# JuliaPhysics/BeamletOptics.jl

Hardware: AMD Instinct MI355X
Metric: ray-surface intersections/s (higher is better)
Workload: dtype f64

## Files before the change

### beamletoptics.jl_amd/csrc/bmo_lane.hpp

```cpp
#pragma once
#include <math.h>
#include <stdint.h>

#include "../../include/bmo.h"
#include "bmo_jlmath.hpp"

#if defined(__HIPCC__)
#define BMO_HD __host__ __device__ __forceinline__
#define BMO_NOUNROLL _Pragma("unroll 1")
#else
#define BMO_HD inline __attribute__((always_inline))
#define BMO_NOUNROLL
#endif

#if !defined(BMO_DUAL_PASSES)
#define BMO_DUAL_PASSES 1
#endif

namespace bmo {

#if defined(BMO_EMU_STATS)
inline long g_emu_sdf_any = 0, g_emu_sdf_leaf = 0, g_emu_normal = 0, g_emu_normal_fd = 0;
#endif

#if defined(__HIP_DEVICE_COMPILE__)
#define BMO_UNIFORM(i) __builtin_amdgcn_readfirstlane(i)
#define BMO_KONST __attribute__((address_space(4)))
__device__ __forceinline__ bool bmo_same_id(int32_t u, int32_t id) {
    asm volatile("" : "+s"(u));
    return u == id;
}
#else
#define BMO_UNIFORM(i) (i)
#define BMO_KONST
inline bool bmo_same_id(int32_t u, int32_t id) { return u == id; }
#endif
#if defined(__HIP_DEVICE_COMPILE__)
#define BMO_WAVE_ALL(p) (__all(p) != 0)
#define BMO_WAVE_ANY(p) (__any(p) != 0)
#else
#define BMO_WAVE_ALL(p) (p)
#define BMO_WAVE_ANY(p) (p)
#endif
typedef const BMO_KONST bmo_shape CShape;
typedef const BMO_KONST bmo_object CObject;
typedef const BMO_KONST double CDouble;
typedef const BMO_KONST int32_t CInt;


struct SceneView {
    CObject* objects;
    CShape* shapes;
    CInt* children;
    CDouble* tris;
    CDouble* n_table;
    CDouble* coefs;
    const BMO_KONST struct Cand* cands;
    int32_t n_objects, n_lambda, n_cands;
    double eps_srf, eps_ray, eps_ins, mt_keps, mt_leps, grad_h;
    int32_t march_iters;
    const BMO_KONST struct BvhNode* bvh_nodes = nullptr;
    CInt* bvh_faces = nullptr;
};

struct d3 {
    double x, y, z;
};
struct Hit {
    double t;
    d3 n;
    int32_t obj, shape;
};

BMO_HD double kinf() { return __builtin_huge_val(); }
BMO_HD bool sgn(double x) { return __builtin_signbit(x); }
BMO_HD bool isnan_(double x) { return x != x; }
BMO_HD Hit no_hit() {
    Hit h;
    h.t = kinf();
    h.n = {0, 0, 0};
    h.obj = -1;
    h.shape = -1;
    return h;
}

BMO_HD double jmax_rule(double x, double y) {
    if (isnan_(x) || isnan_(y)) return x + y;
    return ((y > x) || (sgn(y) < sgn(x))) ? y : x;
}
BMO_HD double jmin_rule(double x, double y) {
    if (isnan_(x) || isnan_(y)) return x + y;
    return ((y < x) || (sgn(y) > sgn(x))) ? y : x;
}
#if defined(__HIP_DEVICE_COMPILE__) && !defined(BMO_RULE_MINMAX)
BMO_HD double jmax(double x, double y) {
    double m;
    asm("v_max_f64 %0, %1, %2" : "=v"(m) : "v"(x), "v"(y));
    return __builtin_isunordered(x, y) ? x + y : m;
}
BMO_HD double jmin(double x, double y) {
    double m;
    asm("v_min_f64 %0, %1, %2" : "=v"(m) : "v"(x), "v"(y));
    return __builtin_isunordered(x, y) ? x + y : m;
}
#else
BMO_HD double jmax(double x, double y) { return jmax_rule(x, y); }
BMO_HD double jmin(double x, double y) { return jmin_rule(x, y); }
#endif
BMO_HD double jabs(double x) { return fabs(x); }
BMO_HD double jsqrt(double x) { return sqrt(x); }
BMO_HD double val(double x) { return x; }

template <int N>
struct DualN {
    double v;
    double p[N];
};
using Dual = DualN<3>;
#define BMO_DN template <int N> BMO_HD
BMO_DN double val(const DualN<N>& x) { return x.v; }
BMO_DN DualN<N> operator+(const DualN<N>& x, const DualN<N>& y) {
    DualN<N> r;
    r.v = x.v + y.v;
    for (int q = 0; q < N; ++q) r.p[q] = x.p[q] + y.p[q];
    return r;
}
BMO_DN DualN<N> operator-(const DualN<N>& x, const DualN<N>& y) {
    DualN<N> r;
    r.v = x.v - y.v;
    for (int q = 0; q < N; ++q) r.p[q] = x.p[q] - y.p[q];
    return r;
}
BMO_DN DualN<N> operator+(const DualN<N>& x, double c) {
    DualN<N> r = x;
    r.v = x.v + c;
    return r;
}
BMO_DN DualN<N> operator+(double c, const DualN<N>& x) {
    DualN<N> r = x;
    r.v = c + x.v;
    return r;
}
BMO_DN DualN<N> operator-(const DualN<N>& x, double c) {
    DualN<N> r = x;
    r.v = x.v - c;
    return r;
}
BMO_DN DualN<N> operator-(double c, const DualN<N>& x) {
    DualN<N> r;
    r.v = c - x.v;
    for (int q = 0; q < N; ++q) r.p[q] = -x.p[q];
    return r;
}
BMO_DN DualN<N> operator-(const DualN<N>& x) {
    DualN<N> r;
    r.v = -x.v;
    for (int q = 0; q < N; ++q) r.p[q] = -x.p[q];
    return r;
}
BMO_DN DualN<N> operator*(const DualN<N>& x, const DualN<N>& y) {
    DualN<N> r;
    r.v = x.v * y.v;
    for (int q = 0; q < N; ++q) r.p[q] = (x.p[q] * y.v) + (y.p[q] * x.v);
    return r;
}
BMO_DN DualN<N> operator*(const DualN<N>& x, double c) {
    DualN<N> r;
    r.v = x.v * c;
    for (int q = 0; q < N; ++q) r.p[q] = x.p[q] * c;
    return r;
}
BMO_DN DualN<N> operator*(double c, const DualN<N>& x) {
    DualN<N> r;
    r.v = c * x.v;
    for (int q = 0; q < N; ++q) r.p[q] = x.p[q] * c;
    return r;
}
BMO_DN DualN<N> operator/(const DualN<N>& x, double c) {
    DualN<N> r;
    r.v = x.v / c;
    for (int q = 0; q < N; ++q) r.p[q] = x.p[q] / c;
    return r;
}
BMO_DN DualN<N> jsqrt(const DualN<N>& x) {
    const double s = sqrt(x.v);
    const double d = 1.0 / (2.0 * s);
    DualN<N> r;
    r.v = s;
    for (int q = 0; q < N; ++q) r.p[q] = x.p[q] * d;
    return r;
}
BMO_DN DualN<N> jabs(const DualN<N>& x) {
    const bool neg = sgn(x.v);
    DualN<N> r;
    r.v = neg ? -x.v : x.v;
    for (int q = 0; q < N; ++q) r.p[q] = neg ? -x.p[q] : x.p[q];
    return r;
}
BMO_DN DualN<N> jmax(const DualN<N>& x, const DualN<N>& y) {
    const bool xw = x.v > y.v;
    DualN<N> r;
    r.v = xw ? x.v : y.v;
    for (int q = 0; q < N; ++q) r.p[q] = xw ? x.p[q] : y.p[q];
    return r;
}
BMO_DN DualN<N> jmin(const DualN<N>& x, const DualN<N>& y) {
    const bool xw = x.v < y.v;
    DualN<N> r;
    r.v = xw ? x.v : y.v;
    for (int q = 0; q < N; ++q) r.p[q] = xw ? x.p[q] : y.p[q];
    return r;
}
BMO_DN DualN<N> jmax(const DualN<N>& x, double y) {
    const bool xw = x.v > y;
    DualN<N> r;
    r.v = xw ? x.v : y;
    for (int q = 0; q < N; ++q) r.p[q] = xw ? x.p[q] : 0.0;
    return r;
}
BMO_DN DualN<N> jmin(const DualN<N>& x, double y) {
    const bool xw = x.v < y;
    DualN<N> r;
    r.v = xw ? x.v : y;
    for (int q = 0; q < N; ++q) r.p[q] = xw ? x.p[q] : 0.0;
    return r;
}

template <class T>
struct v3 {
    T x, y, z;
};

BMO_HD void pin(double& x) {
#if defined(__HIP_DEVICE_COMPILE__) && !defined(BMO_NO_PIN)
    asm volatile("" : "+v"(x));
#else
    (void)x;
#endif
}
template <int N>
BMO_HD void pin(DualN<N>& x) {
    pin(x.v);
}
template <class T>
BMO_HD void pin3(v3<T>& p) {
    pin(p.x);
    pin(p.y);
    pin(p.z);
}
BMO_HD double dot3(const d3& a, const d3& b) { return (a.x * b.x + a.y * b.y) + a.z * b.z; }
BMO_HD double norm3(const d3& a) { return sqrt(dot3(a, a)); }
BMO_HD d3 sub3(const d3& a, const d3& b) { return {a.x - b.x, a.y - b.y, a.z - b.z}; }
BMO_HD d3 neg3(const d3& a) { return {-a.x, -a.y, -a.z}; }
BMO_HD d3 cross3(const d3& a, const d3& b) { return {a.y * b.z - a.z * b.y, a.z * b.x - a.x * b.z, a.x * b.y - a.y * b.x}; }
BMO_HD d3 axpy3(const d3& p, double s, const d3& d) { return {p.x + s * d.x, p.y + s * d.y, p.z + s * d.z}; }
BMO_HD d3 normalize_div(const d3& a) {
    double n = norm3(a);
    return {a.x / n, a.y / n, a.z / n};
}
BMO_HD d3 normalize_inv(const d3& a) {
    double inv = 1.0 / norm3(a);
    return {a.x * inv, a.y * inv, a.z * inv};
}
template <class T>
BMO_HD T norm2(const T& x, const T& y) {
    return jsqrt(x * x + y * y);
}
template <class T>
BMO_HD T norm3t(const T& x, const T& y, const T& z) {
    return jsqrt((x * x + y * y) + z * z);
}

BMO_HD bool isapprox(double x, double y, double atol) {
    double rtol = atol > 0.0 ? 0.0 : 1.4901161193847656e-08;
    if (x == y) return true;
    if (isnan_(x) || isnan_(y) || fabs(x) == kinf() || fabs(y) == kinf()) return false;
    return fabs(x - y) <= fmax(atol, rtol * fmax(fabs(x), fabs(y)));
}

template <class T>
BMO_HD v3<T> to_local(CShape& s, const v3<T>& pt) {
    T dx = pt.x - s.pos[0], dy = pt.y - s.pos[1], dz = pt.z - s.pos[2];
    CDouble* m = s.tdir;
    return {(m[0] * dx + m[1] * dy) + m[2] * dz, (m[3] * dx + m[4] * dy) + m[5] * dz, (m[6] * dx + m[7] * dy) + m[8] * dz};
}

template <class T>
BMO_HD T slab2(const T& dx, const T& dy) {
    T mx = jmax(dx, dy);
    T ax = jmax(dx, 0.0), ay = jmax(dy, 0.0);
    return jmin(mx, 0.0) + norm2(ax, ay);
}


BMO_DN DualN<N> operator/(const DualN<N>& x, const DualN<N>& y) {
    const double ia = 1.0 / y.v, fb = -(x.v / (y.v * y.v));
    DualN<N> r;
    r.v = x.v / y.v;
    for (int q = 0; q < N; ++q) r.p[q] = (x.p[q] * ia) + (y.p[q] * fb);
    return r;
}
BMO_DN DualN<N> operator/(double x, const DualN<N>& y) {
    const double divv = x / y.v, f = -(divv / y.v);
    DualN<N> r;
    r.v = divv;
    for (int q = 0; q < N; ++q) r.p[q] = y.p[q] * f;
    return r;
}
BMO_HD bool lt(double a, double b) { return a < b; }
BMO_DN bool lt(const DualN<N>& a, double b) { return a.v < b; }
BMO_DN bool lt(double a, const DualN<N>& b) { return a < b.v; }
BMO_DN bool lt(const DualN<N>& a, const DualN<N>& b) { return a.v < b.v; }
BMO_HD double lit2(double x) { return x * x; }
BMO_HD double lit3(double x) { return x * x * x; }
BMO_DN DualN<N> lit2(const DualN<N>& x) {
    const double d = 2 * x.v;
    DualN<N> r;
    r.v = x.v * x.v;
    for (int q = 0; q < N; ++q) r.p[q] = x.p[q] * d;
    return r;
}
BMO_DN DualN<N> lit3(const DualN<N>& x) {
    const double d = 3 * (x.v * x.v);
    DualN<N> r;
    r.v = x.v * x.v * x.v;
    for (int q = 0; q < N; ++q) r.p[q] = x.p[q] * d;
    return r;
}
BMO_HD double ipow(double x, int n) {
    if (n == 0) return 1.0;
    if (n == 1) return x;
    if (n == 2) return x * x;
    if (n == 3) return x * x * x;
    double r = 1.0;
    while (n > 0) {
        if (n & 1) r *= x;
        x *= x;
        n >>= 1;
    }
    return r;
}
BMO_DN DualN<N> ipow(const DualN<N>& x, int n) {
    const double ev = ipow(x.v, n);
    const double f = n == 0 ? 0.0 : ipow(x.v, n - 1);
    DualN<N> r;
    r.v = ev;
    for (int q = 0; q < N; ++q) r.p[q] = (n == 0 || x.p[q] == 0) ? 0.0 : (x.p[q] * n) * f;
    return r;
}
BMO_HD double knan() { return kinf() - kinf(); }
BMO_HD double mknan(double) { return knan(); }
BMO_DN DualN<N> mknan(const DualN<N>&) {
    DualN<N> r;
    r.v = knan();
    for (int q = 0; q < N; ++q) r.p[q] = knan();
    return r;
}
BMO_HD double jsign(double x) { return x > 0 ? 1.0 : (x < 0 ? -1.0 : x); }
BMO_HD double clamp01(double x) { return x > 1.0 ? 1.0 : (x < 0.0 ? 0.0 : x); }
BMO_DN DualN<N> clamp01(const DualN<N>& x) {
    DualN<N> r = x;
    if (x.v > 1.0 || x.v < 0.0) {
        r.v = x.v > 1.0 ? 1.0 : 0.0;
        for (int q = 0; q < N; ++q) r.p[q] = 0.0;
    }
    return r;
}
template <class T>
BMO_HD void asph_eval(const T& r, double c, double k, CDouble* a, int na, T& z, T& g) {
    const T r2 = lit2(r);
    const T sa1 = 1 - (1 + k) * (c * c) * r2;
    const double Ri = 1 / c;
    const T sa2 = 1 - lit2(r) * (1 + k) / (Ri * Ri);
    T sum_a = r2 * 0.0, sum_r = r * 0.0;
    BMO_NOUNROLL
    for (int i = 1; i <= na; ++i) {
        const T ta = a[i - 1] * ipow(r2, i);
        const T tr = (2 * i * a[i - 1]) * ipow(r, 2 * (i - 1) + 1);
        sum_a = i == 1 ? ta : sum_a + ta;
        sum_r = i == 1 ? tr : sum_r + tr;
    }
    z = lt(sa1, 0.0) ? mknan(r) : c * r2 / (1 + jsqrt(sa1)) + sum_a;
    if (lt(sa2, 0.0)) {
        g = mknan(r);
    } else {
        const T sq = jsqrt(sa2);
        const T gr = 2 * r / (Ri * (sq + 1)) + lit3(r) * (1 + k) / ((Ri * Ri * Ri) * sq * lit2(sq + 1));
        g = -sum_r - gr;
    }
}
template <class T>
BMO_HD T norm_g(const T& g1) { return jsqrt(lit2(g1) + 1.0 * 1.0); }
template <class T>
BMO_HD T sd_line_segment(const T& px, const T& py, double ax, double ay, double bx, double by) {
    const T pax = px - ax, pay = py - ay;
    const double bax = bx - ax, bay = by - ay;
    const T h = clamp01((pax * bax + pay * bay) / (bax * bax + bay * bay));
    const T ex = pax - h * bax, ey = pay - h * bay;
    return jsqrt(ex * ex + ey * ey);
}
template <class T>
BMO_HD T asph_distance(bool convex, const T& r, const T& z, double c, double k, double d, CDouble* a, int na, double max_sag) {
    const T r2 = lit2(r);
    const double r2_bound = (d / 2) * (d / 2);
    T zv, g;
    double zb, gb;
    asph_eval<T>(r, c, k, a, na, zv, g);
    asph_eval<double>(d / 2, c, k, a, na, zb, gb);
    const T e = r - jsign(val(r)) * d / 2;
    const double ngb = norm_g<double>(gb);
    if (convex) {
        if (isnan_(val(zv)) || isnan_(val(g)) || lt(r2_bound, r2)) {
            T db;
            if (lt(z, zb)) db = jsqrt(lit2(e) + lit2(z - zb));
            else if (lt(zb, z) && lt(z, 0.0)) db = jsqrt(lit2(e));
            else if (lt(0.0, z) && (jsign(c) == 1 && zb < 0)) db = jsqrt(lit2(e) + lit2(z));
            else db = jsqrt(lit2(e) + lit2(z - zb));
            return db / ngb;
        }
        const T da = jabs(z - zv) / norm_g<T>(g);
        if (jsign(c) == 1 && zb < 0) {
            const T s1 = sd_line_segment<T>(r, z, d / 2, zb, d / 2, max_sag) / ngb;
            const T s2 = sd_line_segment<T>(r, z, d / 2, max_sag, -d / 2, max_sag) / ngb;
            const T s3 = sd_line_segment<T>(r, z, -d / 2, max_sag, -d / 2, zb) / ngb;
            const T m = jmin(jmin(jmin(da, s1), s2), s3);
            return (lt(zv, z) && lt(z, max_sag)) ? -m : m;
        }
        const T sdl = sd_line_segment<T>(r, z, d / 2, zb, -d / 2, zb) / ngb;
        if (lt(jsign(c) * zv, jsign(c) * z) && lt(jsign(c) * z, jsign(c) * zb)) return -jmin(sdl, da);
        return jmin(sdl, da);
    }
    if (isnan_(val(zv)) || isnan_(val(g))) {
        T db;
        if (lt(z, 0.0)) db = jsqrt(lit2(e) + lit2(z));
        else if (lt(0.0, z) && lt(z, zb)) db = jsqrt(lit2(e));
        else db = jsqrt(lit2(e) + lit2(z - zb));
        return db / ngb;
    }
    const T da = jabs(z - zv) / norm_g<T>(g);
    if (max_sag > 0 && zb < 0) {
        const T sdl = sd_line_segment<T>(r, z, d / 2, zb, -d / 2, zb) / ngb;
        if (lt(r2_bound, r2)) return sdl;
        if (lt(zb, z) && lt(z, zv)) return -jmin(da, sdl);
        if (zb > 0 && (lt(0.0, z) && lt(z, zv))) return -jmin(da, sdl);
        return jmin(da, sdl);
    }
    const T s1 = sd_line_segment<T>(r, z, d / 2, zb, d / 2, 0.0) / ngb;
    const T s2 = sd_line_segment<T>(r, z, d / 2, 0.0, -d / 2, 0.0) / ngb;
    const T s3 = sd_line_segment<T>(r, z, -d / 2, 0.0, -d / 2, zb) / ngb;
    if (lt(r2_bound, r2)) return jmin(jmin(s1, s2), s3);
    const T m = jmin(jmin(jmin(da, s1), s2), s3);
    if (zb < 0 && (lt(zv, z) && lt(z, 0.0))) return -m;
    if (zb > 0 && (lt(0.0, z) && lt(z, zv))) return -m;
    return m;
}
BMO_HD double asph_leaf(CShape& s, CDouble* coefs, double r, double y) {
    return asph_distance<double>(s.kind == BMO_SHAPE_ASPH_CONVEX, r, y, 1 / s.p[0], s.p[1], s.p[2], coefs + s.child_begin, s.child_count, s.p[3]);
}
BMO_DN DualN<N> asph_leaf(CShape&, CDouble*, const DualN<N>& r, const DualN<N>&) { return mknan(r); }

template <class T, int EXT>
BMO_HD T sdf_leaf(CShape& s, const int kind, const v3<T>& pt, CDouble* coefs) {
    const double P0 = s.p[0], P1 = s.p[1], P2 = s.p[2], P3 = s.p[3];
    v3<T> p = to_local(s, pt);
    const unsigned cls = (unsigned)((0x0005041214032150ull >> (4 * (kind & 15))) & 15ull) * (kind < 16 ? 1u : 0u);
    if (cls == 1) {
        pin3(p);
        double ra, ha, off, sub;
        if (kind == BMO_SHAPE_PLANO) {
            ra = P1 / 2;
            ha = P0 / 2;
            off = P0 / 2;
            sub = 0.0;
        } else if (kind == BMO_SHAPE_CYLINDER) {
            ra = P0;
            ha = P1;
            off = 0.0;
            sub = 0.0;
        } else {
            ra = P1;
            ha = P2;
            off = 0.0;
            sub = P0;
        }
        T r = norm2(p.x, p.z);
        if (kind == BMO_SHAPE_RING) r = r - sub;
        T h = kind == BMO_SHAPE_PLANO ? p.y - off : p.y;
        return slab2(jabs(r) - ra, jabs(h) - ha);
    }
    if (cls == 2) {
        pin3(p);
        double radius = P0, w, height;
        T q1 = norm2(p.x, p.z), q2;
        if (kind == BMO_SHAPE_CONVEX) {
            w = P1 / 2;
            height = P3;
            q2 = -p.y + radius;
        } else {
            height = P1;
            w = P2;
            q2 = p.y;
        }
        double a = val(q1), b = val(q2);
        double sv = jmax((height - radius) * (a * a) + (w * w) * (height + radius - 2 * b), height * a - w * b);
        if (sv < 0) return norm2(q1, q2) - radius;
        if (a < w) return height - q2;
        return norm2(q1 - w, q2 - height);
    }
    if (cls == 3) {
        pin3(p);
        double radius = P0, dia = P1, sag = P2;
        T x0 = p.x + 0.0, z0 = p.z + 0.0;
        T y1 = p.y + sag / 2;
        T r = norm2(x0, z0);
        T sdf1 = slab2(jabs(r) - dia / 2, jabs(y1) - sag / 2);
        T y2 = p.y + radius;
        T sdf2 = norm3t(x0, y2, z0) - radius;
        return jmax(sdf1, -sdf2);
    }
    if (cls == 4) {
        pin3(p);
        T qx = jabs(p.x) - P0, qy = jabs(p.y) - P1, qz = jabs(p.z) - P2;
        T box = norm3t(jmax(qx, 0.0), jmax(qy, 0.0), jmax(qz, 0.0)) + jmin(jmax(qx, jmax(qy, qz)), 0.0);
        if (kind == BMO_SHAPE_BOX) return box;
        T pln = (p.x + p.y) / 1.4142135623730951;
        return jmax(box, pln);
    }
    if constexpr (EXT >= 2) {
        if (kind == BMO_SHAPE_ASPH_CONVEX || kind == BMO_SHAPE_ASPH_CONCAVE) {
            T r = norm2(p.x, p.z) - 0.0;
            return asph_leaf(s, coefs, r, p.y);
        }
    }
    if constexpr (EXT >= 2) {
        if (kind == BMO_SHAPE_ACYL_CONVEX || kind == BMO_SHAPE_ACYL_CONCAVE) {
            const double height = P2;
            T d2 = asph_distance<T>(kind == BMO_SHAPE_ACYL_CONVEX, p.z, p.y, 1 / P0, P3, P1, coefs + s.child_begin, s.child_count, s.p[4]);
            T w2 = jabs(p.x) - height / 2;
            return jmin(jmax(d2, w2), 0.0) + norm2(jmax(d2, 0.0), jmax(w2, 0.0));
        }
        if (kind == BMO_SHAPE_CYL_CONVEX) {
            const double r = P0, dia = P1, height = P2;
            const double h = sqrt(r * r - (dia / 2) * (dia / 2));
            const double w = sqrt(r * r - h * h);
            T q1 = jabs(p.y), q2 = p.z;
            const double a = val(q1), b = val(q2);
            const double sv = jmax((h - r) * (a * a) + (w * w) * (h + r - 2 * b), h * a - w * b);
            T d2 = (sv < 0) ? norm2(q1, q2) - r : ((a < w) ? h - q2 : norm2(q1 - w, q2 - h));
            T w2 = jabs(p.x) - height / 2;
            return jmin(jmax(d2, w2), 0.0) + norm2(jmax(d2, 0.0), jmax(w2, 0.0));
        }
        if (kind == BMO_SHAPE_CYL_CONCAVE) {
            const double radius = P0, dia = P1, height = P2;
            const double ar = fabs(radius);
            const double sg = ar - sqrt(ar * ar - 0.25 * (dia * dia));
            T x0 = p.x + 0.0, z0 = p.z + 0.0;
            T y1 = p.y + (-radius);
            T c = slab2(jabs(norm2(p.z, y1)) - ar, jabs(x0) - height / 2);
            T y2 = p.y + (-sg / 2 * jsign(radius));
            T qx = jabs(x0) - height / 2, qy = jabs(y2) - sg / 2, qz = jabs(z0) - dia / 2;
            T l = norm3t(jmax(qx, 0.0), jmax(qy, 0.0), jmax(qz, 0.0)) + jmin(jmax(qx, jmax(qy, qz)), 0.0);
            return jmax(l, -c);
        }
    }
    if (cls == 5) {
        pin3(p);
        T r = norm3t(p.x, p.y, p.z);
        return kind == BMO_SHAPE_SPHERE ? r - P0 : r;
    }
    return T{} + kinf();
}

template <class T, int EXT>
BMO_HD T sdf_simple(const SceneView& S, CShape& s, const v3<T>& pt) {
    const int kind0 = s.kind;
    const bool men = EXT >= 1 && kind0 == BMO_SHAPE_MENISCUS;
    const int nleaf = men ? 3 : 1;
    T acc = T{};
    BMO_NOUNROLL
    for (int q = 0; q < nleaf; ++q) {
        CShape& leaf = men ? S.shapes[S.children[s.child_begin + q]] : s;
        const T v = sdf_leaf<T, EXT>(leaf, men ? leaf.kind : kind0, men ? to_local(s, pt) : pt, S.coefs);
        if (q == 0) acc = v;
        else if (q == 1) acc = jmin(acc, v);
        else acc = jmax(acc, -v);
    }
    return acc;
}

constexpr int BMO_CC_MAX = 8;
struct ChildCache {
    double* v;
    int stride;
    int prev_best;
    double others_lb = -__builtin_huge_val();
    double acc = 0.0;
    bool valid = false;
};
BMO_HD void child_cache_reset(ChildCache& cc) {
    cc.prev_best = 0;
    cc.others_lb = -kinf();
    cc.acc = 0.0;
    cc.valid = false;
}

struct ShapeHead {
    int32_t kind, child_count, flags;
    int32_t child_begin, tri_begin;
};
BMO_HD ShapeHead shape_head(CShape& s) {
    ShapeHead h;
    h.kind = s.kind;
    h.child_count = s.child_count;
    h.flags = s.flags;
    h.child_begin = s.child_begin;
    h.tri_begin = s.tri_begin;
    return h;
}
template <int EXT>
BMO_HD double sdf_any(const SceneView& S, const ShapeHead& H, CShape& s, const d3& p, int32_t& best_child, ChildCache& cc, double moved) {
#if defined(BMO_EMU_STATS)
    ++g_emu_sdf_any;
#endif
    const v3<double> pt{p.x, p.y, p.z};
    const bool uni = H.kind == BMO_SHAPE_UNION;
    const int nch = uni ? H.child_count : 1;
    double best = kinf();
    best_child = 0;
    const int first = (uni && BMO_UNIFORM(cc.prev_best) < nch) ? BMO_UNIFORM(cc.prev_best) : 0;
    const double acc = cc.acc + (moved * (1.0 + 1e-9) + 1e-12);
    const int32_t sflags = H.flags;
    const bool consecutive = uni && (sflags & BMO_SHAPE_FLAG_CONSECUTIVE);
    const int32_t cb = H.child_begin, first_id = H.tri_begin;
    const bool all_exact = !(sflags & BMO_SHAPE_FLAG_INEXACT);
    double m1 = kinf(), m2 = kinf();
    int i1 = -1;
    BMO_NOUNROLL
    for (int q = 0; q < nch; ++q) {
        const int c = q == 0 ? first : (q <= first ? q - 1 : q);
        CShape& ch = uni ? S.shapes[consecutive ? first_id + c : S.children[cb + c]] : s;
        bool skip = false;
        double lb = -kinf();
        const bool usable = uni && c < BMO_CC_MAX && (all_exact || !(ch.flags & BMO_SHAPE_FLAG_INEXACT));
        if (q > 0 && usable && cc.valid) {
            const double bound = best > 0.0 ? best : 0.0;
            lb = cc.v[c * cc.stride] - acc;
            skip = lb > bound + 1e-12;
        }
        double stored = lb;
        if (!skip) {
#if defined(BMO_EMU_STATS)
            ++g_emu_sdf_leaf;
#endif
            const double v = sdf_simple<double, EXT>(S, ch, pt);
            stored = v;
            if (q == 0) {
                best = v;
                best_child = c;
                if (uni && first == cc.prev_best) {
                    const double bound = v > 0.0 ? v : 0.0;
                    if (cc.others_lb - acc > bound + 1e-12) {
                        cc.acc = acc;
                        return v;
                    }
                }
            } else {
                const bool less = (v < best) || (v == best && sgn(v) && !sgn(best));
                const bool same = (v == best) && (sgn(v) == sgn(best));
                if (less || (same && c < best_child)) best_child = c;
                best = jmin(best, v);
            }
        }
        if (uni && c < BMO_CC_MAX) cc.v[c * cc.stride] = stored;
        const double key = (usable && stored == stored) ? stored : -kinf();
        if (key < m1) {
            m2 = m1;
            m1 = key;
            i1 = c;
        } else if (key < m2) {
            m2 = key;
        }
    }
    if (uni) {
        cc.prev_best = best_child;
        cc.others_lb = (i1 == best_child) ? m2 : m1;
        cc.acc = 0.0;
        cc.valid = true;
    }
    return best;
}

template <int EXT>
BMO_HD d3 normal_of(const SceneView& S, CShape& sh, const d3& p) {
#if !defined(BMO_STUB_NORMAL)
    {
#if defined(BMO_EMU_STATS)
        ++g_emu_normal;
#endif
        double g0 = 0.0, g1 = 0.0, g2 = 0.0;
#if BMO_DUAL_PASSES == 1
        {
            v3<DualN<3>> x{{p.x, {1, 0, 0}}, {p.y, {0, 1, 0}}, {p.z, {0, 0, 1}}};
            const DualN<3> y = sdf_simple<DualN<3>, EXT>(S, sh, x);
            g0 = y.p[0], g1 = y.p[1], g2 = y.p[2];
        }
#elif BMO_DUAL_PASSES == 2
        {
            v3<DualN<2>> x{{p.x, {1, 0}}, {p.y, {0, 1}}, {p.z, {0, 0}}};
            const DualN<2> y = sdf_simple<DualN<2>, EXT>(S, sh, x);
            g0 = y.p[0], g1 = y.p[1];
        }
        {
            v3<DualN<1>> x{{p.x, {0}}, {p.y, {0}}, {p.z, {1}}};
            const DualN<1> y = sdf_simple<DualN<1>, EXT>(S, sh, x);
            g2 = y.p[0];
        }
#else
        BMO_NOUNROLL
        for (int ax = 0; ax < 3; ++ax) {
            v3<DualN<1>> x{{p.x, {ax == 0 ? 1.0 : 0.0}}, {p.y, {ax == 1 ? 1.0 : 0.0}}, {p.z, {ax == 2 ? 1.0 : 0.0}}};
            const DualN<1> y = sdf_simple<DualN<1>, EXT>(S, sh, x);
            g0 = ax == 0 ? y.p[0] : g0;
            g1 = ax == 1 ? y.p[0] : g1;
            g2 = ax == 2 ? y.p[0] : g2;
        }
#endif
        d3 n = normalize_inv(d3{g0, g1, g2});
        if (!isnan_(n.x) && !isnan_(n.y) && !isnan_(n.z)) return n;
#if defined(BMO_EMU_STATS)
        ++g_emu_normal_fd;
#endif
    }
#endif
    const double e = S.grad_h;
    double g0 = 0, g1 = 0, g2 = 0;
    BMO_NOUNROLL
    for (int q = 0; q < 6; ++q) {
        const int ax = q >> 1;
        const bool minus = q & 1;
        double ox = ax == 0 ? e : 0.0, oy = ax == 1 ? e : 0.0, oz = ax == 2 ? e : 0.0;
        v3<double> pt = minus ? v3<double>{p.x - ox, p.y - oy, p.z - oz} : v3<double>{p.x + ox, p.y + oy, p.z + oz};
#if defined(BMO_EMU_STATS)
        ++g_emu_sdf_leaf;
#endif
        double v = sdf_simple<double, EXT>(S, sh, pt);
        if (ax == 0) g0 = minus ? g0 - v : v;
        else if (ax == 1) g1 = minus ? g1 - v : v;
        else g2 = minus ? g2 - v : v;
    }
    return normalize_div(d3{g0, g1, g2});
}
template <int EXT>
BMO_HD d3 normal_at(const SceneView& S, int32_t sid, int32_t kind, int32_t child_begin, const d3& p, int32_t best_child) {
    int32_t tid = sid;
    if (kind == BMO_SHAPE_UNION) tid = S.children[child_begin + best_child];
    d3 n{0, 0, 0};
    for (bool todo = true; todo;) {
        const int32_t u = BMO_UNIFORM(tid);
        if (bmo_same_id(u, tid)) {
            n = normal_of<EXT>(S, S.shapes[u], p);
            todo = false;
        }
    }
    return n;
}

BMO_HD double cull_entry_raw(double cx, double cy, double cz, double R, const d3& pos, const d3& dir);
BMO_HD double cull_entry(CShape& s, const d3& pos, const d3& dir) { return cull_entry_raw(s.bs_center[0], s.bs_center[1], s.bs_center[2], s.bs_radius, pos, dir); }
BMO_HD double cull_entry_raw(double cx, double cy, double cz, double R, const d3& pos, const d3& dir) {
    if (!(R >= 0.0)) return 0.0;
    d3 oc{cx - pos.x, cy - pos.y, cz - pos.z};
    double dd = dot3(dir, dir), b = dot3(oc, dir), cc = dot3(oc, oc), R2 = R * R;
    if (!(cc > R2)) return 0.0;
    if (b < 0.0) return -1.0;
    double disc = b * b - dd * (cc - R2);
    if (disc < 0.0) return -1.0;
    return (b - sqrt(disc)) / dd;
}
struct BoundSphere {
    double cx, cy, cz, R;
};
BMO_HD bool cull_receding(const BoundSphere& b, const d3& pos, const d3& dir) {
    if (!(b.R >= 0.0)) return false;
    d3 co{pos.x - b.cx, pos.y - b.cy, pos.z - b.cz};
    return dot3(co, co) > b.R * b.R && dot3(co, dir) > 0.0;
}

BMO_HD double moeller_trumbore(CDouble* f, const d3& pos, const d3& dir, double keps, double leps) {
    d3 V1{f[0], f[1], f[2]}, V2{f[3], f[4], f[5]}, V3{f[6], f[7], f[8]};
    d3 E1 = sub3(V2, V1), E2 = sub3(V3, V1);
    d3 Pv = cross3(dir, E2);
    double Det = dot3(E1, Pv);
    if (fabs(Det) < keps) return kinf();
    d3 Tv = sub3(pos, V1);
    double invDet = 1 / Det;
    double u = dot3(Tv, Pv) * invDet;
    if ((u < 0 - keps) || (u > 1 + keps)) return kinf();
    d3 Qv = cross3(Tv, E1);
    double v = dot3(dir, Qv) * invDet;
    if ((v < 0 - keps) || (u + v > 1 + keps)) return kinf();
    double t = dot3(E2, Qv) * invDet;
    if (t < leps) return kinf();
    return t;
}

BMO_HD double mesh_nearest(const SceneView& S, int tri0, int ntri, const d3& pos, const d3& dir, int32_t& fid) {
    double t0 = kinf();
    fid = -1;
    BMO_NOUNROLL
    for (int i = 0; i < ntri; ++i) {
        const double t = moeller_trumbore(S.tris + 9 * (tri0 + i), pos, dir, S.mt_keps, S.mt_leps);
        if (t < t0) {
            t0 = t;
            fid = i;
        }
    }
    return t0;
}
struct BvhNode {
    double lo[3], hi[3];
    int32_t first, count, axis, pad;
};
constexpr int BMO_BVH_MAX_DEPTH = 64;
constexpr int BMO_BVH_STACK = BMO_BVH_MAX_DEPTH;

BMO_HD bool bvh_visit(const BMO_KONST BvhNode& n, const double* o, const double* iv, double pad, double tmin, double tb) {
    double tn = -kinf(), tf = kinf();
    bool outside = false;
    for (int k = 0; k < 3; ++k) {
        const double lo = n.lo[k] - pad, hi = n.hi[k] + pad;
        if (fabs(iv[k]) == kinf()) {
            outside = outside || o[k] < lo || o[k] > hi;
        } else {
            const double a = (lo - o[k]) * iv[k], b = (hi - o[k]) * iv[k];
            tn = fmax(tn, fmin(a, b));
            tf = fmin(tf, fmax(a, b));
        }
    }
    return !(outside || tn > tf || tf < tmin || tn > tb);
}

BMO_HD double mesh_nearest_bvh(const SceneView& S, int32_t hdr, int tri0, int ntri, const d3& pos, const d3& dir, double tlim, int32_t& fid) {
    const BMO_KONST BvhNode& H = S.bvh_nodes[hdr];
    const d3 oc{pos.x - H.lo[0], pos.y - H.lo[1], pos.z - H.lo[2]};
    const double D = sqrt(dot3(oc, oc)) + H.hi[0];
    const double pad = D * 0x1p-46 + D * sqrt(dot3(dir, dir)) * H.hi[1];
    if (!(pad < kinf())) return mesh_nearest(S, tri0, ntri, pos, dir, fid);
    const double o[3] = {pos.x, pos.y, pos.z}, iv[3] = {1.0 / dir.x, 1.0 / dir.y, 1.0 / dir.z};
    const double tmin = S.mt_leps >= 0.0 ? 0.0 : -kinf();
    double best = kinf();
    fid = -1;
    int32_t stk[BMO_BVH_STACK];
    int sp = 0;
    int32_t ni = H.first;
    bool tested = false;
    BMO_NOUNROLL
    for (;;) {
        const BMO_KONST BvhNode& nd = S.bvh_nodes[ni];
        const double tb = best < tlim ? best : tlim;
        if (tested || BMO_WAVE_ANY(bvh_visit(nd, o, iv, pad, tmin, tb))) {
            const int32_t first = nd.first, count = nd.count;
            if (count > 0) {
                BMO_NOUNROLL
                for (int i = 0; i < count; ++i) {
                    const int32_t f = S.bvh_faces[first + i];
                    const double t = moeller_trumbore(S.tris + 9 * (tri0 + f), pos, dir, S.mt_keps, S.mt_leps);
                    if (t < best || (t == best && f < fid)) {
                        best = t;
                        fid = f;
                    }
                }
            } else {
                const bool n0 = BMO_WAVE_ANY(bvh_visit(S.bvh_nodes[first], o, iv, pad, tmin, tb));
                const bool n1 = BMO_WAVE_ANY(bvh_visit(S.bvh_nodes[first + 1], o, iv, pad, tmin, tb));
                if (n0 || n1) {
                    int32_t next = n0 ? first : first + 1;
                    if (n0 && n1) {
                        if (sp + 1 > BMO_BVH_STACK) return mesh_nearest(S, tri0, ntri, pos, dir, fid);
                        const int ax = nd.axis;
                        const double da = ax == 0 ? dir.x : (ax == 1 ? dir.y : dir.z);
                        const int32_t back = BMO_UNIFORM((int32_t)(da < 0.0));
                        next = first + (back ? 1 : 0);
                        stk[sp++] = first + (back ? 0 : 1);
                    }
                    ni = next;
                    tested = true;
                    continue;
                }
            }
        }
        if (sp == 0) break;
        ni = BMO_UNIFORM(stk[--sp]);
        tested = false;
    }
    return best;
}

BMO_HD d3 mesh_normal(const SceneView& S, int tri) {
    CDouble* f = S.tris + 9 * tri;
    d3 V1{f[0], f[1], f[2]}, V2{f[3], f[4], f[5]}, V3{f[6], f[7], f[8]};
    d3 n = normalize_div(cross3(sub3(V2, V1), sub3(V3, V1)));
    return normalize_div(n);
}

struct Cand {
    double cx, cy, cz, R;
    int32_t sid, obj;
    int32_t info;
    int32_t pad;
};
enum { CAND_PLATE_SUBSTRATE = 1, CAND_PLATE_COATING = 2 };
inline int fill_candidates(const bmo_object* objects, int n_objects, const bmo_shape* shapes, Cand* out) {
    int n = 0;
    for (int o = 0; o < n_objects; ++o) {
        const bmo_object& ob = objects[o];
        int np = (ob.kind == BMO_OBJ_DOUBLET) ? 2 : (ob.kind == BMO_OBJ_CUBE_BS ? 3 : (ob.kind == BMO_OBJ_PLATE_BS ? 2 : 1));
        if (ob.kind == BMO_OBJ_NONINTERACTABLE) np = 0;
        for (int k = 0; k < np; ++k) {
            int32_t sid = ob.shape[k];
            int32_t info = 0;
            if (ob.kind == BMO_OBJ_PLATE_BS) {
                sid = ob.shape[1 - k];
                info = k == 0 ? CAND_PLATE_COATING : CAND_PLATE_SUBSTRATE;
            }
            if (out) {
                const bmo_shape& sh = shapes[sid];
                out[n] = Cand{sh.bs_center[0], sh.bs_center[1], sh.bs_center[2], sh.bs_radius, sid, o, info, 0};
            }
            ++n;
        }
    }
    return n;
}

constexpr int BMO_LANE_MEM = 11;
struct LaneMem {
    double* m;
    int stride;
    BMO_HD d3 get3(int c) const { return d3{m[c * stride], m[(c + 1) * stride], m[(c + 2) * stride]}; }
    BMO_HD void put3(int c, const d3& v) const {
        m[c * stride] = v.x;
        m[(c + 1) * stride] = v.y;
        m[(c + 2) * stride] = v.z;
    }
};

BMO_HD bool cull_miss(double cx, double cy, double cz, double R, const d3& pos, const d3& dir) {
    const d3 oc{cx - pos.x, cy - pos.y, cz - pos.z};
    const double dd = dot3(dir, dir), b = dot3(oc, dir), cc = dot3(oc, oc), R2 = R * R;
    return (R >= 0.0) & (cc > R2) & ((b < 0.0) | (b * b - dd * (cc - R2) < 0.0));
}

template <int EXT, bool RETR = false>
BMO_HD Hit tracing_step(const SceneView& S, const d3& pos_in, const d3& dir0, int32_t hint_obj, int32_t hint_shape, uint32_t& calls, ChildCache& cc,
                        const LaneMem& lm, bool probe = false, int32_t probe_obj = -1, bool fresh_allowed = true, bool* probe_missed = nullptr) {
    enum { CLASSIFY = 0, INSIDE = 1, OUTSIDE = 2, FINAL = 3 };
    double x_t = kinf();
    int32_t x_shape = -1, x_obj = -1;
    int32_t x_aux = 0;
    bool done = false;
    int32_t skip_obj = -1;
    int32_t tested_shape = -1;
    int32_t coat_obj = -1;
    const int n_obj = S.n_objects, n_cand = S.n_cands;
    lm.put3(3, pos_in);
    BMO_NOUNROLL
    for (int pass = RETR ? 0 : 1; pass <= 2; ++pass) {
        bool in_pass;
        int32_t hs = -1;
        int o_lo = 0, o_hi = n_obj;
        if (pass == 2) {
            in_pass = x_shape >= 0;
        } else if (RETR && pass == 0) {
            in_pass = probe;
            if (in_pass) {
                calls += 1;
                hs = hint_shape;
                if (hint_shape >= 0) {
                    o_hi = 0;
                } else {
                    o_lo = probe_obj;
                    o_hi = probe_obj + 1;
                }
            }
        } else {
            in_pass = !done;
            if (RETR && probe) {
                if (in_pass) {
                    if (probe_missed) *probe_missed = true;
                    if (!fresh_allowed) {
                        in_pass = false;
                    } else {
                        if (hint_shape < 0) skip_obj = probe_obj;
                        calls += (uint32_t)n_obj;
                    }
                }
            } else if (in_pass) {
                hs = hint_shape;
                calls += hs >= 0 ? 1u : (uint32_t)n_obj;
            }
        }
        if (in_pass && hs >= 0) tested_shape = hs;
        const int c_end = pass == 2 ? 0 : n_cand;
        BMO_NOUNROLL
        for (int c0 = 0; c0 == 0 || c0 < c_end; c0 += 64) {
            unsigned long long mask = 0;
            unsigned long long wave_mask = 0;
            const int c1 = c_end - c0 < 64 ? c_end - c0 : 64;
            BMO_NOUNROLL
            for (int q = c0 == 0 ? -1 : -2;;) {
                const int slot = q < 0 ? -1 : c0 + q;
                bool take = false;
                int32_t sid = 0, info = 0, obj = -1;
                if (q == -1) {
                    take = in_pass && (pass == 2 || hs >= 0);
                    sid = pass == 2 ? x_shape : hs;
                } else if (q >= 0) {
                    take = ((mask >> q) & 1ull) != 0;
                    const BMO_KONST Cand& cd = S.cands[slot];
                    sid = cd.sid;
                    obj = cd.obj;
                    info = cd.info;
                }
                for (bool todo = take; todo;) {
                    const int32_t usid = BMO_UNIFORM(sid);
                    if (!bmo_same_id(usid, sid)) continue;
                    todo = false;
                    bool active = true;
                    CShape& s = S.shapes[usid];
                    const int32_t s_kind = s.kind, s_flags = s.flags;
                    double lim = kinf();
                    d3 pos{0, 0, 0};
                    if (pass != 2) {
                        pos = lm.get3(3);
                        if (slot < 0) {
                            if (cull_miss(s.bs_center[0], s.bs_center[1], s.bs_center[2], s.bs_radius, pos, dir0)) active = false;
                        } else if (x_shape >= 0) {
                            lim = x_t + 1e-6 * (1.0 + x_t);
                            const double t_lb = cull_entry(s, pos, dir0);
                            if (t_lb * (1.0 - 1e-9) - 1e-9 > lim) active = false;
                        }
                    }
                    auto offer = [&](double t, int32_t a, const d3& p) {
                        bool accept = x_shape < 0 || t < x_t;
                        if (info & CAND_PLATE_COATING) {
                            lm.m[6 * lm.stride] = t;
                            coat_obj = obj;
                        }
                        if ((info & CAND_PLATE_SUBSTRATE) && coat_obj == obj) {
                            const double t_coat = lm.m[6 * lm.stride];
                            if (isapprox(t_coat, t, 0.0) || t_coat < t) accept = false;
                        }
                        if (accept) {
                            x_t = t;
                            x_shape = usid;
                            x_obj = slot < 0 ? hint_obj : obj;
                            x_aux = a;
                            lm.put3(0, p);
                            if (slot < 0) done = true;
                        }
                    };
                    if (s_kind == BMO_SHAPE_MESH) {
                        if (pass == 2) {
                            lm.put3(0, mesh_normal(S, s.tri_begin + x_aux));
                        } else if (active) {
                            int32_t fid = -1;
                            double t;
                            if constexpr (EXT >= 3) {
                                if (s_flags & BMO_SHAPE_FLAG_BVH) {
                                    const double tlim = (x_shape >= 0 && !(info & CAND_PLATE_COATING)) ? x_t : kinf();
                                    t = mesh_nearest_bvh(S, s.child_begin, s.tri_begin, s.tri_count, pos, dir0, tlim, fid);
                                } else {
                                    t = mesh_nearest(S, s.tri_begin, s.tri_count, pos, dir0, fid);
                                }
                            } else {
                                t = mesh_nearest(S, s.tri_begin, s.tri_count, pos, dir0, fid);
                            }
                            if (fid >= 0) offer(t, fid, d3{0, 0, 0});
                        }
                        active = false;
                    }
                    if (BMO_WAVE_ANY(active)) {
                        const ShapeHead H{s_kind, s.child_count, s_flags, s.child_begin, s.tri_begin};
                        const bool exact = !(s_flags & BMO_SHAPE_FLAG_INEXACT);
                        enum { ST_BACK = 4, ST_PENDING = 8, ST_ACTIVE = 16 };
                        int st = (active ? ST_ACTIVE : 0) | (pass == 2 ? (FINAL | ST_PENDING) : CLASSIFY);
                        int32_t bc = 0;
                        if (pass == 2) {
                            pos = lm.get3(0);
                            bc = x_aux;
                        }
                        BMO_NOUNROLL
                        for (int round = 0; round < 2; ++round) {
                            double dist = 0.0, t0 = 0.0, t_in = 0.0;
                            int it = 1;
                            child_cache_reset(cc);
                            while ((st & (ST_ACTIVE | ST_PENDING)) == ST_ACTIVE) {
                                const int phase = st & 3;
                                double moved = 0.0;
                                if (phase == INSIDE) {
                                    pos = axpy3(pos, S.eps_ins, dir0);
                                    t_in += S.eps_ins;
                                    moved = S.eps_ins;
                                } else if (phase == OUTSIDE) {
                                    pos = axpy3(pos, (st & ST_BACK) ? -dist : dist, dir0);
                                    moved = fabs(dist);
                                }
                                const double d = sdf_any<EXT>(S, H, s, pos, bc, cc, moved);
                                if (phase == OUTSIDE) {
                                    const bool growing = d > dist;
                                    dist = d;
                                    t0 += d;
                                    it += 1;
                                    if (d < S.eps_ray) {
                                        offer((st & ST_BACK) ? t_in - t0 : t0, bc, pos);
                                        st = 0;
                                    } else {
                                        bool recede = false;
                                        if (growing) {
                                        const double R = s.bs_radius;
                                        const d3 co{pos.x - s.bs_center[0], pos.y - s.bs_center[1], pos.z - s.bs_center[2]};
                                        const double cd = dot3(co, dir0);
                                        recede = R >= 0.0 && dot3(co, co) > R * R && ((st & ST_BACK) ? cd < 0.0 : cd > 0.0);
                                        }
                                        if (recede || (exact && !(st & ST_BACK) && t0 > lim)
                                            || !(it <= S.march_iters))
                                            st = 0;
                                    }
                                } else if (phase == CLASSIFY) {
                                    if (d > S.eps_srf) {
                                        st = ST_ACTIVE | OUTSIDE;
                                        dist = d;
                                        t0 = d;
                                        it = 1;
                                        if (!(it <= S.march_iters) || (exact && t0 > lim)) st = 0;
                                    } else {
                                        st |= ST_PENDING;
                                    }
                                } else {
                                    if (d > 0) {
                                        st = ST_ACTIVE | ST_BACK | OUTSIDE;
                                        dist = d;
                                        t0 = d;
                                        it = 1;
                                    } else {
                                        it += 1;
                                    }
                                    if (!(it <= S.march_iters)) st = 0;
                                }
                            }
                            if (!BMO_WAVE_ANY(st & ST_ACTIVE)) break;
                            if (st & ST_ACTIVE) {
                                const d3 n = normal_at<EXT>(S, usid, s_kind, H.child_begin, pos, bc);
                                if ((st & 3) == FINAL) {
                                    lm.put3(0, n);
                                    st = 0;
                                } else if (dot3(dir0, n) <= 0 && 1 <= S.march_iters) {
                                    st = ST_ACTIVE | INSIDE;
                                } else {
                                    st = 0;
                                }
                            }
                        }
                    }
                }
                if (slot < 0 && pass == 1 && take && !done) calls += (uint32_t)n_obj;
                if (q < 0) {
                    if (pass == 2) break;
                    const bool collect = in_pass && !done && o_lo < o_hi;
                    if (c1 > 0 && BMO_WAVE_ANY(collect)) {
                        const d3 p0 = lm.get3(3);
                        BMO_NOUNROLL
                        for (int i0 = 0; i0 < c1; i0 += 4) {
                            bool want[4];
                            const BMO_KONST Cand* cp = S.cands + (c0 + i0);
                            for (int u = 0; u < 4; ++u) {
                                const BMO_KONST Cand& cd = cp[u];
                                const int32_t co = cd.obj, cs = cd.sid;
                                const bool in_range = RETR ? ((co >= o_lo) & (co < o_hi) & (co != skip_obj)) : true;
                                want[u] = (i0 + u < c1) & collect & in_range & (cs != tested_shape) & !cull_miss(cd.cx, cd.cy, cd.cz, cd.R, p0, dir0);
                            }
                            for (int u = 0; u < 4; ++u) {
                                mask |= (unsigned long long)want[u] << (i0 + u);
                                if (BMO_WAVE_ANY(want[u])) wave_mask |= 1ull << (i0 + u);
                            }
                        }
                    }
                } else {
                    wave_mask &= ~(1ull << q);
                }
                if (!wave_mask) break;
                q = (int)__builtin_ctzll(wave_mask);
            }
        }
        if (RETR && pass == 0 && x_shape >= 0) done = true;
    }
    Hit X;
    X.t = x_t;
    X.obj = x_obj;
    X.shape = x_shape;
    X.n = x_shape >= 0 ? lm.get3(0) : d3{0, 0, 0};
    return X;
}

BMO_HD d3 reflection3d(const d3& dir, const d3& n) {
    double k = 2 * dot3(dir, n);
    return {dir.x - k * n.x, dir.y - k * n.y, dir.z - k * n.z};
}
BMO_HD bool refraction3d(const d3& dir, const d3& normal, double n1, double n2, d3& out, bool& tir) {
    if (!isapprox(norm3(dir), 1.0, 0.0)) return false;
    if (!isapprox(norm3(normal), 1.0, 0.0)) return false;
    double n = n1 / n2;
    double ci = -dot3(normal, dir);
    double st2 = (n * n) * (1 - ci * ci);
    if (st2 > 1.0) {
        out = reflection3d(dir, normal);
        tir = true;
        return true;
    }
    double ct = sqrt(1 - st2);
    double k = n * ci - ct;
    out = {n * dir.x + k * normal.x, n * dir.y + k * normal.y, n * dir.z + k * normal.z};
    tir = false;
    return true;
}

struct cx {
    double re, im;
};
BMO_HD cx cadd(cx a, cx b) { return {a.re + b.re, a.im + b.im}; }
BMO_HD cx csub(cx a, cx b) { return {a.re - b.re, a.im - b.im}; }
BMO_HD cx cneg(cx a) { return {-a.re, -a.im}; }
BMO_HD cx cmul(cx a, cx b) { return {a.re * b.re - a.im * b.im, a.re * b.im + a.im * b.re}; }
BMO_HD cx rmul(double s, cx a) { return {s * a.re, s * a.im}; }
BMO_HD cx cmulr(cx a, double s) { return {a.re * s, a.im * s}; }
BMO_HD cx cdiv(cx a, cx b) {
    double den = b.re * b.re + b.im * b.im;
    return {(a.re * b.re + a.im * b.im) / den, (a.im * b.re - a.re * b.im) / den};
}
BMO_HD double cabs2(cx a) { return a.re * a.re + a.im * a.im; }

struct RayS {
    d3 pos, dir;
    double n;
    cx E0[3];
};

enum StepOutcome { OUT_MISS = 0, OUT_STOP = 1, OUT_CONTINUE = 2, OUT_SPLIT = 3 };

struct StepOut {
    int outcome;
    int status;
    int32_t hint_obj, hint_shape;
    RayS next;
    RayS refl;
    int det_slot;
    double* det;
};

BMO_HD double n_medium(const SceneView& S, int medium, int li) { return S.n_table[medium * S.n_lambda + li]; }

BMO_HD bool isparallel3d(const d3& a, const d3& b) { return isapprox(fabs(dot3(normalize_div(a), normalize_div(b))), 1.0, 2.220446049250313e-16); }

BMO_HD d3 perpendicular_to(const d3& in) {
    double nn = norm3(in);
    d3 nw = fabs(in.x) > 0.9 * nn ? d3{0, 1, 0} : d3{1, 0, 0};
    double k = dot3(nw, in), n2 = nn * nn;
    nw = {nw.x - k * in.x / n2, nw.y - k * in.y / n2, nw.z - k * in.z / n2};
    return normalize_div(nw);
}

BMO_HD void mat3_apply(const cx* P, const cx* v, cx* res) {
    for (int i = 0; i < 3; ++i) res[i] = cadd(cadd(cmul(P[3 * i + 0], v[0]), cmul(P[3 * i + 1], v[1])), cmul(P[3 * i + 2], v[2]));
}

BMO_HD void global_E0(const d3& in, const d3& out, const d3& normal, cx j11, cx j22, const cx* E0, cx* res) {
    bool par = isparallel3d(in, out);
    d3 v = par ? normal : out;
    if (isparallel3d(in, normal)) v = perpendicular_to(in);
    d3 s = normalize_div(cross3(in, v));
    d3 p1 = cross3(in, s);
    double Oin[9] = {s.x, s.y, s.z, p1.x, p1.y, p1.z, in.x, in.y, in.z};
    double Oo[9];
    d3 mo = neg3(out);
    bool anti = norm3(sub3(in, mo)) <= 1.4901161193847656e-08 * fmax(norm3(in), norm3(mo));
    d3 c1 = p1, c2 = in;
    if (!(par && !anti)) {
        c1 = cross3(out, s);
        c2 = out;
    }
    Oo[0] = s.x; Oo[1] = c1.x; Oo[2] = c2.x;
    Oo[3] = s.y; Oo[4] = c1.y; Oo[5] = c2.y;
    Oo[6] = s.z; Oo[7] = c1.z; Oo[8] = c2.z;
    cx J[9] = {j11, {0, 0}, {0, 0}, {0, 0}, j22, {0, 0}, {0, 0}, {0, 0}, {1, 0}};
    cx A[9], P[9];
    for (int i = 0; i < 3; ++i)
        for (int j = 0; j < 3; ++j)
            A[3 * i + j] = cadd(cadd(rmul(Oo[3 * i + 0], J[0 + j]), rmul(Oo[3 * i + 1], J[3 + j])), rmul(Oo[3 * i + 2], J[6 + j]));
    for (int i = 0; i < 3; ++i)
        for (int j = 0; j < 3; ++j)
            P[3 * i + j] = cadd(cadd(cmulr(A[3 * i + 0], Oin[0 + j]), cmulr(A[3 * i + 1], Oin[3 + j])), cmulr(A[3 * i + 2], Oin[6 + j]));
    mat3_apply(P, E0, res);
}
BMO_HD bool e0_orthogonal(const d3& dir, const cx* E0) {
    cx d = cadd(cadd(rmul(dir.x, E0[0]), rmul(dir.y, E0[1])), rmul(dir.z, E0[2]));
    return sqrt(cabs2(d)) <= 1e-14;
}
BMO_HD void fresnel(double theta, double n, cx& rs, cx& rp, cx& ts, cx& tp) {
    double ct = jl::cos(theta), st = jl::sin(theta);
    double x = n * n - st * st;
    cx r = x >= 0.0 ? cx{sqrt(x), 0.0} : cx{0.0, sqrt(-x)};
    cx c{ct, 0};
    rs = cdiv(csub(c, r), cadd(c, r));
    cx n2c{(n * n) * ct, 0};
    rp = cdiv(cadd(cx{-(n * n) * ct, 0}, r), cadd(n2c, r));
    ts = cadd(rs, cx{1, 0});
    tp = cdiv(cx{2 * n * ct, 0}, cadd(n2c, r));
}
BMO_HD double angle3d(const d3& a, const d3& b) {
    double arg = dot3(a, b) / (norm3(a) * norm3(b));
    arg = arg < -1.0 ? -1.0 : (arg > 1.0 ? 1.0 : arg);
    return jl::acos(arg);
}

BMO_HD d3 hit_point(const RayS& r, double t) { return axpy3(r.pos, t, r.dir); }

struct NextInOut {
    StepOut& o;
    BMO_HD void put(const d3& pos, const d3& dir, double n) const {
        o.next.pos = pos;
        o.next.dir = dir;
        o.next.n = n;
    }
};
template <int KIND, class NextSink>
BMO_HD void interact(const SceneView& S, const RayS& ray, const Hit& X, int li, double lambda, double opl_before, StepOut& o,
                     const NextSink& sink, int ent_override = -1) {
    CObject& ob = S.objects[X.obj];
    o.outcome = OUT_STOP;
    o.hint_obj = o.hint_shape = -1;
    o.det_slot = -1;
    enum { A_STOP = 0, A_REFLECT, A_REFRACT, A_SPLIT, A_SPOT, A_PSF, A_POLARIZER };
    int action = A_STOP;
    int medium = -1;
    int32_t hshape = -1;
    int32_t force_hobj = -1;
    int32_t force_hshape = -1;
    int split_mode = 0;
    switch (ob.kind) {
        case BMO_OBJ_MIRROR: action = A_REFLECT; break;
        case BMO_OBJ_REFRACTIVE:
            action = A_REFRACT;
            medium = ob.medium[0];
            hshape = ob.shape[0];
            break;
        case BMO_OBJ_DOUBLET: {
            if (KIND != BMO_BEAM_RAY) break;
            int part = X.shape == ob.shape[0] ? 0 : 1;
            action = A_REFRACT;
            medium = ob.medium[part];
            hshape = ob.shape[part];
            force_hobj = X.obj;
            force_hshape = ob.shape[1 - part];
            break;
        }
        case BMO_OBJ_THIN_BS: action = A_SPLIT; break;
        case BMO_OBJ_PLATE_BS:
            if (X.shape == ob.shape[0]) {
                action = A_REFRACT;
                medium = ob.medium[0];
                hshape = ob.shape[0];
                force_hobj = X.obj;
                force_hshape = ob.shape[1];
            } else if (X.shape == ob.shape[1]) {
                action = A_SPLIT;
                split_mode = 1;
            }
            break;
        case BMO_OBJ_CUBE_BS:
            if (X.shape == ob.shape[2]) {
                action = A_SPLIT;
                split_mode = 2;
            } else {
                int part = X.shape == ob.shape[0] ? 0 : 1;
                action = A_REFRACT;
                medium = ob.medium[part];
                hshape = ob.shape[part];
                force_hobj = X.obj;
                force_hshape = ob.shape[2];
            }
            break;
        case BMO_OBJ_SPOTDETECTOR: action = A_SPOT; break;
        case BMO_OBJ_PSFDETECTOR:
            if (KIND != BMO_BEAM_POLARIZED) action = A_PSF;
            break;
        case BMO_OBJ_POLARIZER:
            if (KIND == BMO_BEAM_POLARIZED) action = A_POLARIZER;
            break;
        default: break;
    }

    const d3 hp = hit_point(ray, X.t);
    if (action == A_REFLECT || action == A_REFRACT) {
        d3 nd;
        double n_out = ray.n;
        cx j11{-1, 0}, j22{1, 0};
        int32_t ho = -1, hs = -1;
        if (action == A_REFLECT) {
            nd = reflection3d(ray.dir, X.n);
        } else {
            d3 normal = X.n;
// ... 518 lines not shown
```

Before: 42.42 billion.

## Add specialized fast-path sphere-march loop for union shapes with cached best child

Adds an inner fast-march loop for union shapes in the outside phase. While the child-cache lower bound proves the previously best child still dominates, it evaluates only that child's leaf SDF, specialised per leaf class at compile time. This skips the general sdf_any loop overhead and the runtime dispatch on leaf kind. When the loop exits, the precomputed value is handed to sdf_any so that step is not evaluated twice. The cost is more code, extra register pressure, and a switch per entry into the loop.

Measured after the change: 44.68 billion (median of 6 runs). +5.3%, better.

```diff
diff --git a/beamletoptics.jl_amd/csrc/bmo_lane.hpp b/beamletoptics.jl_amd/csrc/bmo_lane.hpp
--- a/beamletoptics.jl_amd/csrc/bmo_lane.hpp
+++ b/beamletoptics.jl_amd/csrc/bmo_lane.hpp
@@ -16,11 +16,15 @@
 #if !defined(BMO_DUAL_PASSES)
 #define BMO_DUAL_PASSES 1
 #endif
+#if !defined(BMO_MARCH_FASTPATH)
+#define BMO_MARCH_FASTPATH 1
+#endif
 
 namespace bmo {
 
 #if defined(BMO_EMU_STATS)
 inline long g_emu_sdf_any = 0, g_emu_sdf_leaf = 0, g_emu_normal = 0, g_emu_normal_fd = 0;
+inline long g_emu_union = 0, g_emu_union_fast = 0, g_emu_union_loop = 0;
 #endif
 
 #if defined(__HIP_DEVICE_COMPILE__)
@@ -459,11 +463,16 @@
 }
 BMO_DN DualN<N> asph_leaf(CShape&, CDouble*, const DualN<N>& r, const DualN<N>&) { return mknan(r); }
 
-template <class T, int EXT>
+BMO_HD unsigned leaf_class(int kind) { return (unsigned)((0x0005041214032150ull >> (4 * (kind & 15))) & 15ull) * (kind < 16 ? 1u : 0u); }
+template <int C>
+struct LeafClass {
+    static constexpr int value = C;
+};
+template <class T, int EXT, int CLS = 0>
 BMO_HD T sdf_leaf(CShape& s, const int kind, const v3<T>& pt, CDouble* coefs) {
     const double P0 = s.p[0], P1 = s.p[1], P2 = s.p[2], P3 = s.p[3];
     v3<T> p = to_local(s, pt);
-    const unsigned cls = (unsigned)((0x0005041214032150ull >> (4 * (kind & 15))) & 15ull) * (kind < 16 ? 1u : 0u);
+    const unsigned cls = CLS != 0 ? (unsigned)CLS : leaf_class(kind);
     if (cls == 1) {
         pin3(p);
         double ra, ha, off, sub;
@@ -526,13 +535,13 @@
         T pln = (p.x + p.y) / 1.4142135623730951;
         return jmax(box, pln);
     }
-    if constexpr (EXT >= 2) {
+    if constexpr (EXT >= 2 && CLS == 0) {
         if (kind == BMO_SHAPE_ASPH_CONVEX || kind == BMO_SHAPE_ASPH_CONCAVE) {
             T r = norm2(p.x, p.z) - 0.0;
             return asph_leaf(s, coefs, r, p.y);
         }
     }
-    if constexpr (EXT >= 2) {
+    if constexpr (EXT >= 2 && CLS == 0) {
         if (kind == BMO_SHAPE_ACYL_CONVEX || kind == BMO_SHAPE_ACYL_CONCAVE) {
             const double height = P2;
             T d2 = asph_distance<T>(kind == BMO_SHAPE_ACYL_CONVEX, p.z, p.y, 1 / P0, P3, P1, coefs + s.child_begin, s.child_count, s.p[4]);
@@ -618,12 +627,16 @@
     return h;
 }
 template <int EXT>
-BMO_HD double sdf_any(const SceneView& S, const ShapeHead& H, CShape& s, const d3& p, int32_t& best_child, ChildCache& cc, double moved) {
+BMO_HD double sdf_any(const SceneView& S, const ShapeHead& H, CShape& s, const d3& p, int32_t& best_child, ChildCache& cc, double moved,
+                      bool has_pre = false, double pre_v = 0.0) {
 #if defined(BMO_EMU_STATS)
     ++g_emu_sdf_any;
 #endif
     const v3<double> pt{p.x, p.y, p.z};
     const bool uni = H.kind == BMO_SHAPE_UNION;
+#if defined(BMO_EMU_STATS)
+    g_emu_union += uni;
+#endif
     const int nch = uni ? H.child_count : 1;
     double best = kinf();
     best_child = 0;
@@ -652,7 +665,7 @@
 #if defined(BMO_EMU_STATS)
             ++g_emu_sdf_leaf;
 #endif
-            const double v = sdf_simple<double, EXT>(S, ch, pt);
+            const double v = (has_pre && c == cc.prev_best) ? pre_v : sdf_simple<double, EXT>(S, ch, pt);
             stored = v;
             if (q == 0) {
                 best = v;
@@ -660,6 +673,9 @@
                 if (uni && first == cc.prev_best) {
                     const double bound = v > 0.0 ? v : 0.0;
                     if (cc.others_lb - acc > bound + 1e-12) {
+#if defined(BMO_EMU_STATS)
+                        ++g_emu_union_fast;
+#endif
                         cc.acc = acc;
                         return v;
                     }
@@ -1094,9 +1110,63 @@
                         for (int round = 0; round < 2; ++round) {
                             double dist = 0.0, t0 = 0.0, t_in = 0.0;
                             int it = 1;
+                            bool has_pre = false;
+                            double pre_v = 0.0;
                             child_cache_reset(cc);
                             while ((st & (ST_ACTIVE | ST_PENDING)) == ST_ACTIVE) {
                                 const int phase = st & 3;
+                                if constexpr (BMO_MARCH_FASTPATH == 2 || (BMO_MARCH_FASTPATH == 1 && EXT == 0 && !RETR)) {
+                                    if (H.kind == BMO_SHAPE_UNION && phase == OUTSIDE) {
+                                        const int32_t fb = BMO_UNIFORM(cc.prev_best);
+                                        if (cc.prev_best == fb && fb < H.child_count) {
+                                            CShape& ch = S.shapes[(H.flags & BMO_SHAPE_FLAG_CONSECUTIVE) ? H.tri_begin + cc.prev_best
+                                                                                                         : S.children[H.child_begin + cc.prev_best]];
+                                            const int ck = ch.kind;
+                                            auto fast_march = [&](auto cls_tag) {
+                                                constexpr int CLS = decltype(cls_tag)::value;
+                                                BMO_NOUNROLL
+                                                for (;;) {
+                                                    const bool back = (st & ST_BACK) != 0;
+                                                    const d3 np = axpy3(pos, back ? -dist : dist, dir0);
+                                                    const double acc = cc.acc + (fabs(dist) * (1.0 + 1e-9) + 1e-12);
+                                                    const double v = sdf_leaf<double, EXT, CLS>(ch, ck, v3<double>{np.x, np.y, np.z}, S.coefs);
+                                                    const double bound = v > 0.0 ? v : 0.0;
+                                                    const double t1 = t0 + v;
+                                                    const int it1 = it + 1;
+                                                    bool go = (cc.others_lb - acc > bound + 1e-12) && !(v < S.eps_ray) && !(exact && !back && t1 > lim) &&
+                                                              (it1 <= S.march_iters);
+                                                    if (go && v > dist) {
+                                                        const double R = s.bs_radius;
+                                                        const d3 co{np.x - s.bs_center[0], np.y - s.bs_center[1], np.z - s.bs_center[2]};
+                                                        const double cd = dot3(co, dir0);
+                                                        go = !(R >= 0.0 && dot3(co, co) > R * R && (back ? cd < 0.0 : cd > 0.0));
+                                                    }
+                                                    if (!go) {
+                                                        has_pre = true;
+                                                        pre_v = v;
+                                                        break;
+                                                    }
+#if defined(BMO_EMU_STATS)
+                                                    ++g_emu_sdf_any, ++g_emu_sdf_leaf, ++g_emu_union, ++g_emu_union_fast, ++g_emu_union_loop;
+#endif
+                                                    pos = np;
+                                                    cc.acc = acc;
+                                                    dist = v;
+                                                    t0 = t1;
+                                                    it = it1;
+                                                }
+                                            };
+                                            switch (leaf_class(ck)) {
+                                                case 1: fast_march(LeafClass<1>{}); break;
+                                                case 2: fast_march(LeafClass<2>{}); break;
+                                                case 3: fast_march(LeafClass<3>{}); break;
+                                                case 4: fast_march(LeafClass<4>{}); break;
+                                                case 5: fast_march(LeafClass<5>{}); break;
+                                                default: break;
+                                            }
+                                        }
+                                    }
+                                }
                                 double moved = 0.0;
                                 if (phase == INSIDE) {
                                     pos = axpy3(pos, S.eps_ins, dir0);
@@ -1106,7 +1176,8 @@
                                     pos = axpy3(pos, (st & ST_BACK) ? -dist : dist, dir0);
                                     moved = fabs(dist);
                                 }
-                                const double d = sdf_any<EXT>(S, H, s, pos, bc, cc, moved);
+                                const double d = sdf_any<EXT>(S, H, s, pos, bc, cc, moved, has_pre, pre_v);
+                                has_pre = false;
                                 if (phase == OUTSIDE) {
                                     const bool growing = d > dist;
                                     dist = d;
```
